# facebookresearch/VideoPose3D

Measured on NVIDIA H100. Metric: frames/sec (arc 3,3,3,3,3, T=243, N=1024), higher is better.
Workload: dtype fp16 (IEEE fp16 operands and activations, fp32 accumulate)

## Files before the change

videopose3d_b200/csrc/conv_gemm.cu:

```cuda
#include "conv_gemm.cuh"

#include <stdlib.h>
#include <string.h>

#include <type_traits>

#include "ptx.cuh"

namespace vp3d {

enum class Epi { kTrain, kGeneral, kLean };
enum class Fmt { kRuntime, kBf16, kF16, kI8 };
enum class Sched { kCooperative, kPingPong };
enum class U8Out { kNone, kBeside, kAlone };

struct InstKey {
  int block_n;
  Epi epi;
  Fmt fmt;
  Sched sched;
  bool res;
  bool out2;
  U8Out u8;
  constexpr bool operator==(const InstKey& o) const {
// ... 85 lines not shown
  const uint32_t q = quant_u8(v0, inv_s) | (quant_u8(v1, inv_s) << 8);
  asm volatile("st.shared.u16 [%0], %1;" ::"r"(addr), "h"((unsigned short)q) : "memory");
}

__device__ __forceinline__ void slab_reduce(float (&s)[8][2], float (&q)[8][2], float* s_pair,
                                            int lane, int wq, uint32_t bar_id) {
#pragma unroll
  for (int off = 4; off <= 16; off <<= 1) {
#pragma unroll
    for (int jj = 0; jj < 8; ++jj) {
#pragma unroll
      for (int e = 0; e < 2; ++e) {
        s[jj][e] += __shfl_xor_sync(0xffffffffu, s[jj][e], off);
        q[jj][e] += __shfl_xor_sync(0xffffffffu, q[jj][e], off);
      }
    }
  }
  if ((wq & 1) && lane < 4) {
#pragma unroll
    for (int jj = 0; jj < 8; ++jj) {
      *reinterpret_cast<float2*>(s_pair + 8 * jj + 2 * lane) = make_float2(s[jj][0], s[jj][1]);
      *reinterpret_cast<float2*>(s_pair + 64 + 8 * jj + 2 * lane) = make_float2(q[jj][0], q[jj][1]);
    }
  }
  named_bar_sync(bar_id, 64);
  if (!(wq & 1) && lane < 4) {
#pragma unroll
    for (int jj = 0; jj < 8; ++jj) {
      const float2 so = *reinterpret_cast<const float2*>(s_pair + 8 * jj + 2 * lane);
      const float2 qo = *reinterpret_cast<const float2*>(s_pair + 64 + 8 * jj + 2 * lane);
      s[jj][0] += so.x; s[jj][1] += so.y;
      q[jj][0] += qo.x; q[jj][1] += qo.y;
    }
  }
  named_bar_sync(bar_id, 64);
}

#ifdef VP3D_TIMELINE
__device__ __forceinline__ void tl_stamp(const ConvGemmArgs& p, int ev) {
  if (!p.timeline) return;
  int slot;
  if (blockIdx.x == 0) slot = 0;
  else if (blockIdx.x == gridDim.x - 1) slot = 1;
  else return;
  unsigned long long g;
  asm volatile("mov.u64 %0, %%globaltimer;" : "=l"(g));
  p.timeline[(slot * 32 + ev) * 2] = g;
  p.timeline[(slot * 32 + ev) * 2 + 1] = (unsigned long long)clock64();
}
#define TL(ev) tl_stamp(p, ev)
#else
#define TL(ev) ((void)0)
#endif

template <int BLOCK_N, Fmt FMT, int H, class Acc>
__device__ __forceinline__ void wgmma_kblock(Acc (&acc)[H][BLOCK_N / 2], const uint64_t (&da)[H],
                                             uint64_t db, bool first) {
#pragma unroll
  for (int h = 0; h < H; ++h) {
#pragma unroll
    for (int k = 0; k < 4; ++k) {
      const uint32_t accumulate = (first && k == 0) ? 0u : 1u;
      if constexpr (FMT == Fmt::kI8) {
        if constexpr (BLOCK_N == 128) wgmma_m64n128k32_u8s8(acc[h], da[h] + 2 * k, db + 2 * k, accumulate);
        else wgmma_m64n64k32_u8s8(acc[h], da[h] + 2 * k, db + 2 * k, accumulate);
      } else if constexpr (BLOCK_N == 128) {
        if constexpr (FMT == Fmt::kF16) wgmma_m64n128_f16(acc[h], da[h] + 2 * k, db + 2 * k, accumulate);
        else wgmma_m64n128_bf16(acc[h], da[h] + 2 * k, db + 2 * k, accumulate);
      } else {
        if constexpr (FMT == Fmt::kF16) wgmma_m64n64_f16(acc[h], da[h] + 2 * k, db + 2 * k, accumulate);
        else wgmma_m64n64_bf16(acc[h], da[h] + 2 * k, db + 2 * k, accumulate);
      }
    }
  }
}

template <class I, int H, class Issued>
__device__ __forceinline__ void mma_tile(typename I::Acc (&acc)[H][I::kBlockN / 2],
                                         const ConvGemmArgs& p, bool f16, uint32_t smem_a,
                                         uint32_t a_off, uint32_t smem_b, uint32_t full_bar,
                                         uint32_t empty_bar, uint32_t& stage_io, uint32_t& phase_io,
                                         int k_iters, int lane, bool tl_first, Issued issued) {
  uint32_t stage = stage_io, phase = phase_io;
  uint32_t prev_stage = 0;
  for (int it = 0; it < k_iters; ++it) {
    mbar_wait(full_bar + stage * 8, phase);
#ifdef VP3D_TIMELINE
    if (tl_first && it == 0) TL(4);
#endif
    const uint32_t a_st = smem_a + stage * I::kABytes + a_off;
    uint64_t da[H];
#pragma unroll
    for (int h = 0; h < H; ++h) da[h] = make_gmma_desc_sw128(a_st + h * 64 * 128, 16, 1024);
    const uint64_t db = make_gmma_desc_sw128(smem_b + stage * I::kBBytes, 16, 1024);
#pragma unroll
    for (int h = 0; h < H; ++h) wgmma_fence_operands(acc[h]);
    wgmma_fence();
    if constexpr (I::kFmt != Fmt::kRuntime) wgmma_kblock<I::kBlockN, I::kFmt>(acc, da, db, it == 0);
    else if (f16) wgmma_kblock<I::kBlockN, Fmt::kF16>(acc, da, db, it == 0);
    else wgmma_kblock<I::kBlockN, Fmt::kBf16>(acc, da, db, it == 0);
    wgmma_commit();
#pragma unroll
    for (int h = 0; h < H; ++h) wgmma_fence_operands(acc[h]);
    if (it > 0) {
      wgmma_wait<1>();
#pragma unroll
      for (int h = 0; h < H; ++h) wgmma_fence_operands(acc[h]);
      if (lane == 0) mbar_arrive(empty_bar + prev_stage * 8);
    }
    prev_stage = stage;
    if (++stage == I::kStages) { stage = 0; phase ^= 1; }
  }
  stage_io = stage; phase_io = phase;
  issued();
  wgmma_wait<0>();
#pragma unroll
  for (int h = 0; h < H; ++h) wgmma_fence_operands(acc[h]);
  if (k_iters > 0 && lane == 0) mbar_arrive(empty_bar + prev_stage * 8);
}

template <class I>
__global__ void __launch_bounds__(384, 1)
conv_gemm_kernel(const __grid_constant__ CUtensorMap tmap_a,
                 const __grid_constant__ CUtensorMap tmap_w,
                 const __grid_constant__ CUtensorMap tmap_out,
                 const __grid_constant__ CUtensorMap tmap_res,
                 const __grid_constant__ CUtensorMap tmap_z, const ConvGemmArgs p) {
  using Acc = typename I::Acc;
  constexpr int kBlocksPerTile = I::kBlockN / 64;
  constexpr int kFrag = I::kBlockN / 2;
  constexpr int kBK = I::kI8 ? kBlockK8 : kBlockK;

  extern __shared__ uint8_t smem_raw[];
  const uint32_t raw_addr = smem_u32(smem_raw);
  const uint32_t base = (raw_addr + 1023u) & ~1023u;
  uint8_t* smem = smem_raw + (base - raw_addr);

  const uint32_t smem_a = base;
  const uint32_t smem_b = base + I::kStages * I::kABytes;
  const uint32_t smem_store = base + I::kStages * I::kStageBytes;
  const uint32_t smem_res = smem_store + I::kStagingBytes;
  const uint32_t smem_u8 = smem_res + I::kResSlots * I::kTileBytes;
  const uint32_t bar_base = smem_u8 + I::kU8Bytes;
  const uint32_t full_bar = bar_base;
  const uint32_t empty_bar = bar_base + I::kStages * 8;
  const uint32_t rfull_bar = bar_base + 2 * I::kStages * 8;
  const uint32_t rempty_bar = rfull_bar + 32;
  const uint32_t dep_bar = rempty_bar + 32;
  const uint32_t affine_off = (dep_bar + 8 - base + 15u) & ~15u;
  float* s_affine = reinterpret_cast<float*>(smem + affine_off);
  float* s_pairs = reinterpret_cast<float*>(smem + affine_off + I::kAffineBytes);

  const int warp = threadIdx.x >> 5;
  const int lane = threadIdx.x & 31;
  if (threadIdx.x == 0) TL(0);

  const int m_tiles = p.dilated ? p.samples * p.tiles_per_sample : p.tiles_per_sample;
  const int total_tiles = m_tiles * p.n_tiles;
  const int k_iters = p.pairs * p.taps * p.kblocks_per_tap;
  const bool has_res = (p.flags & kEpiResidual) != 0;
  const bool bnb = I::kTrain && p.bnb != 0;
  const int aux_tiles = (has_res ? p.res_planes : 0) + (bnb ? 1 : 0);
  const int res_stages =
      (aux_tiles > 0 && I::kResSlots >= aux_tiles) ? I::kResSlots / aux_tiles : 1;

  if (warp == 0 && lane == 0) {
    tma_prefetch_desc(&tmap_a);
    tma_prefetch_desc(&tmap_w);
    tma_prefetch_desc(&tmap_out);
    if (I::kRes) tma_prefetch_desc(&tmap_res);
    if (I::kRes && bnb) tma_prefetch_desc(&tmap_z);
    if (I::kU8) tma_prefetch_desc(&tmap_z);
  }
  if (warp == 1 && lane == 0) {
    for (int s = 0; s < I::kStages; ++s) {
      mbar_init(full_bar + s * 8, 1);
      mbar_init(empty_bar + s * 8, I::kPP ? 4 : 8);
    }
    for (int s = 0; s < 4; ++s) {
      mbar_init(rfull_bar + s * 8, 1);
      mbar_init(rempty_bar + s * 8, I::kPP ? 1 : 256);
    }
    mbar_init(dep_bar, 1);
    fence_mbar_init();
  }
  __syncthreads();
  if (threadIdx.x == 0) TL(1);
  if (warp != 0) {
    griddep_wait();
    griddep_launch_dependents();
  }
  if (threadIdx.x == 32) {
    mbar_arrive(dep_bar);
    TL(2);
  }

  if (warp == 0) {
    if (lane == 0) {
      constexpr bool kEarlyW = !I::kTrain;
      if (!kEarlyW) mbar_wait(dep_bar, 0);
      const int n_pre = kEarlyW ? (k_iters < I::kStages ? k_iters : I::kStages) : 0;
      int mode = n_pre > 0 ? 0 : 2;
      if (kEarlyW && mode == 2) mbar_wait(dep_bar, 0);
      int w = blockIdx.x;
      if (w < total_tiles) {
        int n_blk, sample, row0;
        tile_coords(p, w, n_blk, sample, row0);
        uint32_t stage = 0, phase = 0;
        int it = 0, pair = 0, tap = 0, kb = 0;
        for (;;) {
          const int a_plane = (pair == 1) ? 1 : 0;
          const int w_plane = (pair == 2) ? 1 : 0;
          const uint32_t fb = full_bar + stage * 8;
          if (mode != 1) {
            mbar_wait(empty_bar + stage * 8, phase ^ 1);
            mbar_expect_tx(fb, I::kStageBytes);
            const int w_row = (w_plane * p.taps + tap) * p.n_pad + n_blk * I::kBlockN;
            tma_load_2d(&tmap_w, fb, smem_b + stage * I::kBBytes, kb * kBK, w_row);
          }
          if (mode != 0) {
            const int a_row = row0 + tap * p.tap_row_step;
            const int a_col = tap * p.tap_col_step + kb * kBK;
            tma_load_4d(&tmap_a, fb, smem_a + stage * I::kABytes, a_col, a_row, sample, a_plane);
#ifdef VP3D_TIMELINE
            if (w == (int)blockIdx.x && it == 0) TL(3);
#endif
          }
          if (++stage == I::kStages) { stage = 0; phase ^= 1; }
          ++it;
          if (++kb == p.kblocks_per_tap) {
            kb = 0;
            if (++tap == p.taps) { tap = 0; ++pair; }
          }
          if (mode == 0 && it == n_pre) {
            mbar_wait(dep_bar, 0);
            mode = 1;
            it = 0; pair = 0; tap = 0; kb = 0;
            stage = 0; phase = 0;
          } else if (mode == 1 && it == n_pre) {
            mode = 2;
          }
          if (it == k_iters) {
            w += gridDim.x;
            if (w >= total_tiles) break;
            tile_coords(p, w, n_blk, sample, row0);
            it = 0; pair = 0; tap = 0; kb = 0;
          }
        }
      }
    }
  } else if (warp == 1) {
    if (I::kPP && I::kRes && lane == 0) {
      uint32_t filled[2] = {0u, 0u};
      for (int j = 0, w = blockIdx.x; w < total_tiles; ++j, w += gridDim.x) {
        int n_blk, sample, row0;
        tile_coords(p, w, n_blk, sample, row0);
        const int g = j & 1;
        for (int sb = 0; sb < kBlocksPerTile; ++sb) {
          const uint32_t n = g ? filled[1] : filled[0];
          const uint32_t slot = 2u * g + (n & 1u);
          mbar_wait(rempty_bar + slot * 8, ((n >> 1) & 1u) ^ 1u);
          mbar_expect_tx(rfull_bar + slot * 8, I::kTileBytes);
          tma_load_4d(&tmap_res, rfull_bar + slot * 8, smem_res + slot * I::kTileBytes,
                      n_blk * I::kBlockN + sb * 64 + p.res_tma_col_off, row0 + p.res_tma_row_off,
                      sample, 0);
          if (g) ++filled[1];
          else ++filled[0];
        }
      }
    } else if (!I::kPP && I::kRes && lane == 0) {
      uint32_t rs = 0, rphase = 0;
      for (int w = blockIdx.x; w < total_tiles; w += gridDim.x) {
        int n_blk, sample, row0;
        tile_coords(p, w, n_blk, sample, row0);
        for (int sb = 0; sb < kBlocksPerTile; ++sb) {
          const int col = n_blk * I::kBlockN + sb * 64;
          const bool res_here = has_res && col >= p.res_col_begin && col < p.res_col_begin + p.res_cols;
          if (!res_here && !bnb) continue;
          const int n_res = res_here ? p.res_planes : 0;
          mbar_wait(rempty_bar + rs * 8, rphase ^ 1);
          mbar_expect_tx(rfull_bar + rs * 8, (n_res + (bnb ? 1 : 0)) * I::kTileBytes);
          const uint32_t slot0 = smem_res + rs * aux_tiles * I::kTileBytes;
          for (int pl = 0; pl < n_res; ++pl)
            tma_load_4d(&tmap_res, rfull_bar + rs * 8, slot0 + pl * I::kTileBytes,
                        col - p.res_col_begin + p.res_tma_col_off, row0 + p.res_tma_row_off, sample,
                        pl);
          if (bnb)
            tma_load_4d(&tmap_z, rfull_bar + rs * 8, slot0 + (aux_tiles - 1) * I::kTileBytes, col,
                        row0, sample, 0);
          if (++rs == (uint32_t)res_stages) { rs = 0; rphase ^= 1; }
        }
      }
    }
  } else if (I::kPP && warp >= 4) {
    const int wg = (warp - 4) >> 2;
    const int wq = warp & 3;
    const int tid = (int)threadIdx.x - 128 - 128 * wg;
    const int rl0 = 16 * wq + (lane >> 2);
    const int cq = 2 * (lane & 3);
    const uint32_t bar_wg = 2u + (uint32_t)wg;
    const uint32_t bar_mine = 8u + (uint32_t)wg, bar_other = 9u - (uint32_t)wg;
    const uint32_t staging = smem_store + wg * I::kTileBytes;
    uint32_t res_seen = 0;
    Acc acc[2][kFrag];
#pragma unroll
    for (int i = 0; i < kFrag; ++i) acc[0][i] = acc[1][i] = 0.0f;

    for (int j = wg, w = blockIdx.x + wg * gridDim.x; w < total_tiles; j += 2, w += 2 * gridDim.x) {
      int n_blk, sample, row0;
      tile_coords(p, w, n_blk, sample, row0);

      const uint32_t fill = (uint32_t)j * (uint32_t)k_iters;
      uint32_t stage = fill % I::kStages, phase = (fill / I::kStages) & 1u;
      if (j > 0) named_bar_sync(bar_mine, 256);
      mma_tile<I>(acc, p, I::kF16, smem_a, 0u, smem_b, full_bar, empty_bar, stage, phase, k_iters,
                  lane, warp == 4 && lane == 0 && w == (int)blockIdx.x, [&] {
                    if (w + (int)gridDim.x < total_tiles) named_bar_arrive(bar_other, 256);
                  });
#ifdef VP3D_TIMELINE
      if (warp == 4 && lane == 0) { if (w == (int)blockIdx.x) TL(7); TL(8); }
#endif

      const float* scale = p.scale + n_blk * I::kBlockN;
      const float* shift = p.shift + n_blk * I::kBlockN;
#pragma unroll
      for (int sb = 0; sb < kBlocksPerTile; ++sb) {
        const int cb = n_blk * I::kBlockN + sb * 64;
        uint32_t tile_smem;
        if constexpr (I::kRes) {
          const uint32_t slot = 2u * wg + (res_seen & 1u);
          mbar_wait(rfull_bar + slot * 8, (res_seen >> 1) & 1u);
          ++res_seen;
          tile_smem = smem_res + slot * I::kTileBytes;
          if constexpr (I::kU8) {
            if (tid == 0) tma_store_wait_read<0>();
            named_bar_sync(bar_wg, 128);
          }
        } else {
          if (tid == 0) tma_store_wait_read<0>();
          named_bar_sync(bar_wg, 128);
          tile_smem = staging;
        }
        const uint32_t u8_tile = I::kU8Alone ? staging : smem_u8 + (uint32_t)wg * (kBlockM * 64);
#pragma unroll
        for (int jj = 0; jj < 8; ++jj) {
          const int j4 = 4 * (sb * 8 + jj);
          const int cl = sb * 64 + jj * 8 + cq;
          const float2 sc = __ldg(reinterpret_cast<const float2*>(scale + cl));
          const float2 sh = __ldg(reinterpret_cast<const float2*>(shift + cl));
#pragma unroll
          for (int h2 = 0; h2 < 2; ++h2) {
#pragma unroll
            for (int h = 0; h < 2; ++h) {
              float v0 = fmaxf(fmaf(static_cast<float>(acc[h2][j4 + 2 * h]), sc.x, sh.x), 0.0f);
              float v1 = fmaxf(fmaf(static_cast<float>(acc[h2][j4 + 2 * h + 1]), sc.y, sh.y), 0.0f);
              const uint32_t off = sw128_off(64 * h2 + rl0 + 8 * h, jj * 8 + cq);
              if (I::kRes) add_pair(v0, v1, ld_shared_u32(tile_smem + off), I::kF16);
              if constexpr (I::kStore16)
                st_shared_u32(tile_smem + off, I::kF16 ? pack_f16x2(v0, v1) : pack_bf16x2(v0, v1));
              if constexpr (I::kU8)
                st_u8_pair(u8_tile + (uint32_t)(64 * h2 + rl0 + 8 * h) * 64u + jj * 8 + cq, v0, v1,
                           p.u8_inv_s);
            }
          }
        }
        fence_proxy_async_smem();
        named_bar_sync(bar_wg, 128);
        if (tid == 0) {
#pragma unroll
          for (int hb = 0; hb < 4; ++hb) {
            if constexpr (I::kStore16)
              tma_store_4d(&tmap_out, tile_smem + hb * 4096u, cb, row0 + 32 * hb, sample, 0);
            if constexpr (I::kU8)
              tma_store_4d(&tmap_z, u8_tile + hb * 2048u, cb, row0 + 32 * hb, sample, 0);
          }
          tma_store_commit();
        }
      }
      if (I::kRes && tid == 0) {
        tma_store_wait_read<0>();
#pragma unroll
        for (int sb = 0; sb < kBlocksPerTile; ++sb)
          mbar_arrive(rempty_bar + (2u * wg + ((res_seen - kBlocksPerTile + sb) & 1u)) * 8);
      }
#ifdef VP3D_TIMELINE
      if (warp == 4 && lane == 0) { if (w == (int)blockIdx.x) TL(9); TL(10); }
#endif
    }
    if (tid == 0) tma_store_wait_all<0>();
#ifdef VP3D_TIMELINE
    if (warp == 4 && lane == 0) TL(11);
#endif
  } else if (!I::kPP && warp >= 4) {
    const int wg = (warp - 4) >> 2;
    const int wq = warp & 3;
    const int tid = (int)threadIdx.x - 128 - 128 * wg;
    const int rl0 = 16 * wq + (lane >> 2);
    const int cq = 2 * (lane & 3);
    const uint32_t bar_wg = 2u + (uint32_t)wg;
    const uint32_t bar_slab = 4u + (uint32_t)(wg * 2 + (wq >> 1));
    float* s_pair = s_pairs + (wg * 2 + (wq >> 1)) * 128;
    const bool f16 = I::kLean ? I::kF16 : p.f16 != 0;
    const bool do_relu = I::kLean || (p.flags & kEpiRelu);
    const bool do_res = I::kLean ? I::kRes : (p.flags & kEpiResidual) != 0;
    const bool do_stats = I::kTrain && (p.flags & kEpiStats);
    const bool do_f32 = !I::kLean && (p.flags & kEpiOutF32);
    const bool do_affine = I::kLean || (p.flags & kEpiAffine);
    const bool two_planes = I::kOut2 && p.out_planes == 2;
    uint32_t stage = 0, phase = 0;
    uint32_t ablock = 0;
    uint32_t sbuf = 0;
    int aff_n_blk = -1;
    Acc acc[1][kFrag];
#pragma unroll
    for (int i = 0; i < kFrag; ++i) acc[0][i] = 0.0f;

    for (int w = blockIdx.x; w < total_tiles; w += gridDim.x) {
      int n_blk, sample, row0;
      tile_coords(p, w, n_blk, sample, row0);
      const int m_blk = w / p.n_tiles;

      mma_tile<I>(acc, p, f16, smem_a, wg * 64 * 128, smem_b, full_bar, empty_bar, stage, phase,
                  k_iters, lane, warp == 4 && lane == 0 && w == (int)blockIdx.x, [] {});
#ifdef VP3D_TIMELINE
      if (warp == 4 && lane == 0) { if (w == (int)blockIdx.x) TL(7); TL(8); }
#endif

      if (do_affine && n_blk != aff_n_blk) {
        named_bar_sync(1, 256);
        const int e = (int)threadIdx.x - 128;
        if (e < I::kBlockN) {
          s_affine[e] = __ldg(p.scale + n_blk * I::kBlockN + e);
          s_affine[I::kBlockN + e] = __ldg(p.shift + n_blk * I::kBlockN + e);
        }
        named_bar_sync(1, 256);
        aff_n_blk = n_blk;
      }

      int t_in[2];
      bool valid[2];
      long long out_row[2], res_row[2];
      bool res_ok[2];
#pragma unroll
      for (int h = 0; h < 2; ++h) {
        const int rt = 64 * wg + rl0 + 8 * h;
        t_in[h] = row0 + rt;
        valid[h] = t_in[h] < p.out_rows;
        out_row[h] = (long long)sample * p.out_rows + t_in[h];
        res_row[h] = 0;
        res_ok[h] = valid[h];
        if (!I::kRes) {
          int rsmp = sample, rtt = t_in[h];
          if (!p.dilated && p.res_sample_div > 0) {
            rsmp = t_in[h] / p.res_sample_div;
            rtt = t_in[h] - rsmp * p.res_sample_div;
          }
          const long long in_sample = (long long)rtt * p.res_row_step + p.res_row_off;
          if (p.res_check_rows && (in_sample < 0 || in_sample >= p.res_rows_per_sample)) res_ok[h] = false;
          res_row[h] = (long long)rsmp * p.res_rows_per_sample + in_sample;
        }
      }
      const bool two_planes_t =
          two_planes && (p.dilated || (row0 < p.lo_row_end && row0 + kBlockM > p.lo_row_begin));

#pragma unroll
      for (int sb = 0; sb < kBlocksPerTile; ++sb) {
        const int cb = n_blk * I::kBlockN + sb * 64;
        const bool res_here = do_res && cb >= p.res_col_begin && cb < p.res_col_begin + p.res_cols;
        const bool aux_here = I::kRes && (res_here || bnb);
        const uint32_t rs = aux_here ? ablock % (uint32_t)res_stages : 0u;
        const uint32_t rphase = aux_here ? (ablock / (uint32_t)res_stages) & 1u : 0u;
        if (aux_here) {
          ++ablock;
          mbar_wait(rfull_bar + rs * 8, rphase);
        }
        const uint32_t aux0 = smem_res + (rs * aux_tiles) * I::kTileBytes;
        const uint32_t my_store = smem_store + (wg * 2 + sbuf) * (I::kOut2 ? 2 : 1) * I::kHalfBytes;
        const uint32_t my_u8 = I::kU8Alone ? my_store : smem_u8 + (uint32_t)(wg * 2 + sbuf) * (64 * 64);
        if (!do_f32) {
          if (tid == 0) tma_store_wait_read<1>();
          named_bar_sync(bar_wg, 128);
        }
        float ss[8][2], sq[8][2];
#pragma unroll
        for (int jj = 0; jj < 8; ++jj) {
          const int j = sb * 8 + jj;
          const int cl = sb * 64 + jj * 8 + cq;
          const int c = cb + jj * 8 + cq;
          float v[2][2] = {{static_cast<float>(acc[0][4 * j]), static_cast<float>(acc[0][4 * j + 1])},
                           {static_cast<float>(acc[0][4 * j + 2]), static_cast<float>(acc[0][4 * j + 3])}};
          if (do_affine) {
            const float2 sc = *reinterpret_cast<const float2*>(s_affine + cl);
            const float2 sh = *reinterpret_cast<const float2*>(s_affine + I::kBlockN + cl);
#pragma unroll
            for (int h = 0; h < 2; ++h) {
              v[h][0] = fmaf(v[h][0], sc.x, sh.x);
              v[h][1] = fmaf(v[h][1], sc.y, sh.y);
            }
          }
          if (do_relu) {
#pragma unroll
            for (int h = 0; h < 2; ++h) { v[h][0] = fmaxf(v[h][0], 0.0f); v[h][1] = fmaxf(v[h][1], 0.0f); }
          }
          if (I::kRes) {
            if (res_here) {
#pragma unroll
              for (int h = 0; h < 2; ++h) {
                const uint32_t off = sw128_off(64 * wg + rl0 + 8 * h, jj * 8 + cq);
                add_pair(v[h][0], v[h][1], ld_shared_u32(aux0 + off), f16);
                for (int pl = 1; pl < p.res_planes; ++pl)
                  add_pair(v[h][0], v[h][1], ld_shared_u32(aux0 + pl * I::kTileBytes + off), false);
              }
            }
          } else if (res_here) {
#pragma unroll
            for (int h = 0; h < 2; ++h) {
              if (!res_ok[h]) continue;
              const __nv_bfloat16* rp = p.res + res_row[h] * p.res_ld + (c - p.res_col_begin);
#pragma unroll
              for (int pl = 0; pl < 2; ++pl) {
                if (pl < p.res_planes) {
                  const uint32_t u = __ldg(reinterpret_cast<const unsigned int*>(rp + pl * p.res_plane_stride));
                  add_pair(v[h][0], v[h][1], u, f16 && pl == 0);
                }
              }
            }
          }
          if (do_f32) {
#pragma unroll
            for (int h = 0; h < 2; ++h) {
              if (!valid[h]) continue;
              float* op = p.out_f32 + out_row[h] * p.out_f32_ld + c;
              if (c < p.n_valid) op[0] = v[h][0];
              if (c + 1 < p.n_valid) op[1] = v[h][1];
            }
          } else {
            if constexpr (I::kU8) {
#pragma unroll
              for (int h = 0; h < 2; ++h)
                st_u8_pair(my_u8 + (uint32_t)(rl0 + 8 * h) * 64u + jj * 8 + cq, v[h][0], v[h][1],
                           p.u8_inv_s);
            }
#pragma unroll
            for (int h = 0; h < 2 && I::kStore16; ++h) {
              const uint32_t hi = f16 ? pack_f16x2(v[h][0], v[h][1]) : pack_bf16x2(v[h][0], v[h][1]);
              const uint32_t off = sw128_off(rl0 + 8 * h, jj * 8 + cq);
              st_shared_u32(my_store + off, hi);
              if (two_planes_t) {
                const uint32_t lo = pack_bf16x2(v[h][0] - bf16_lo_to_f(hi), v[h][1] - bf16_hi_to_f(hi));
                st_shared_u32(my_store + I::kHalfBytes + off, lo);
              }
            }
          }
          if (I::kRes && bnb) {
            const int ch = c % p.bnb_c;
            const bool drop = p.bnb_p > 0.0f;
            const uint32_t thresh = (uint32_t)(p.bnb_p * 65536.0f);
            const float inv_keep = drop ? 1.0f / (1.0f - p.bnb_p) : 1.0f;
            ss[jj][0] = ss[jj][1] = sq[jj][0] = sq[jj][1] = 0.0f;
#pragma unroll
            for (int h = 0; h < 2; ++h) {
              const uint32_t zu =
                  ld_shared_u32(aux0 + (aux_tiles - 1) * I::kTileBytes + sw128_off(64 * wg + rl0 + 8 * h, jj * 8 + cq));
              const float z2[2] = {bf16_lo_to_f(zu), bf16_hi_to_f(zu)};
              const int c0 = c & ~31;
              const unsigned long long elem0 = (unsigned long long)out_row[h] * p.out_ld + c0;
              const uint32_t key = p.bnb_seed_lo ^ (p.bnb_seed_hi * 0x7F4A7C15u) ^
                                   (p.bnb_layer * 0x632BE5ABu) ^
                                   ((uint32_t)((elem0 >> 1) >> 32) * 0x85EBCA77u);
              float m[2] = {1.0f, 1.0f};
              if (drop) {
                uint32_t hh = ((uint32_t)(elem0 >> 1) + (uint32_t)((c - c0) >> 1)) * 0x9E3779B1u + key;
                hh ^= hh >> 16; hh *= 0x85EBCA6Bu; hh ^= hh >> 13; hh *= 0xC2B2AE35u; hh ^= hh >> 16;
                m[0] = ((hh & 0xFFFFu) >= thresh) ? inv_keep : 0.0f;
                m[1] = ((hh >> 16) >= thresh) ? inv_keep : 0.0f;
              }
#pragma unroll
              for (int e = 0; e < 2; ++e) {
                const float g = __bfloat162float(__float2bfloat16_rn(v[h][e]));
                const float y = fmaf(z2[e], __ldg(p.bnb_scale + ch + e), __ldg(p.bnb_shift + ch + e));
                float dy = (valid[h] && y > 0.0f) ? g : 0.0f;
                dy *= m[e];
                ss[jj][e] += dy;
                sq[jj][e] += dy * (z2[e] - __ldg(p.bnb_mean + ch + e));
              }
            }
          } else if (do_stats) {
#pragma unroll
            for (int e = 0; e < 2; ++e) {
              const float x0 = valid[0] ? v[0][e] : 0.0f;
              const float x1 = valid[1] ? v[1][e] : 0.0f;
              ss[jj][e] = x0 + x1;
              sq[jj][e] = x0 * x0 + x1 * x1;
            }
          }
        }
        if (I::kRes && aux_here) mbar_arrive(rempty_bar + rs * 8);
        if (I::kTrain && ((I::kRes && bnb) || do_stats)) {
          slab_reduce(ss, sq, s_pair, lane, wq, bar_slab);
          if (!(wq & 1) && lane < 4) {
            float* sp = ((I::kRes && bnb) ? p.bnb_sums : p.stats) +
                        ((size_t)(m_blk * 4 + 2 * wg + (wq >> 1)) * 2) * p.n_pad + cb + 2 * lane;
#pragma unroll
            for (int jj = 0; jj < 8; ++jj) {
              sp[8 * jj] = ss[jj][0];
              sp[8 * jj + 1] = ss[jj][1];
              sp[p.n_pad + 8 * jj] = sq[jj][0];
              sp[p.n_pad + 8 * jj + 1] = sq[jj][1];
            }
          }
        }
        if (!do_f32) {
          fence_proxy_async_smem();
          named_bar_sync(bar_wg, 128);
          if (tid == 0) {
#pragma unroll
            for (int hb = 0; hb < 2; ++hb) {
              const int r = row0 + 64 * wg + 32 * hb;
              if constexpr (I::kStore16) tma_store_4d(&tmap_out, my_store + hb * 4096u, cb, r, sample, 0);
              if constexpr (I::kU8) tma_store_4d(&tmap_z, my_u8 + hb * 2048u, cb, r, sample, 0);
              if (two_planes_t) tma_store_4d(&tmap_out, my_store + I::kHalfBytes + hb * 4096u, cb, r, sample, 1);
            }
            tma_store_commit();
          }
          sbuf ^= 1u;
        }
      }
#ifdef VP3D_TIMELINE
      if (warp == 4 && lane == 0) { if (w == (int)blockIdx.x) TL(9); TL(10); }
#endif
    }
    if (tid == 0) tma_store_wait_all<0>();
#ifdef VP3D_TIMELINE
    if (warp == 4 && lane == 0) TL(11);
#endif
  }
}

static int g_pdl = -1;
static bool pdl_enabled() {
  if (g_pdl < 0) {
    const char* e = getenv("VP3D_PDL");
    g_pdl = (e && e[0] == '0') ? 0 : 1;
  }
  return g_pdl != 0;
}
void conv_gemm_set_pdl(int on) { g_pdl = on ? 1 : 0; }
bool conv_gemm_pdl_enabled() { return pdl_enabled(); }

static int conv_tiles(const ConvGemmArgs& a) {
  const int m_tiles = a.dilated ? a.samples * a.tiles_per_sample : a.tiles_per_sample;
  return m_tiles * a.n_tiles;
}

template <class I>
static cudaError_t launch_impl(const CUtensorMap& tmap_a, const CUtensorMap& tmap_w,
                               const CUtensorMap& tmap_out, const CUtensorMap& tmap_res,
                               const CUtensorMap& tmap_z, const ConvGemmArgs& args, int num_sms,
                               cudaStream_t stream) {
  auto kernel = conv_gemm_kernel<I>;
  static bool attr_set[kMaxDevices] = {};
  int dev = 0;
  cudaError_t e = cudaGetDevice(&dev);
  if (e != cudaSuccess) return e;
  if (dev < 0 || dev >= kMaxDevices) return cudaErrorInvalidDevice;
  if (!attr_set[dev]) {
    e = cudaFuncSetAttribute(kernel, cudaFuncAttributeMaxDynamicSharedMemorySize, I::kSmemBytes);
    if (e != cudaSuccess) return e;
    attr_set[dev] = true;
  }
  const int total = conv_tiles(args);
  if (total <= 0) return cudaSuccess;
  const int workers = total < num_sms ? total : num_sms;
  cudaLaunchConfig_t cfg;
  memset(&cfg, 0, sizeof(cfg));
  cfg.gridDim = dim3(workers, 1, 1);
  cfg.blockDim = dim3(384, 1, 1);
  cfg.dynamicSmemBytes = I::kSmemBytes;
  cfg.stream = stream;
  cudaLaunchAttribute attr[1];
  int n_attr = 0;
  if (pdl_enabled()) {
    attr[n_attr].id = cudaLaunchAttributeProgrammaticStreamSerialization;
    attr[n_attr].val.programmaticStreamSerializationAllowed = 1;
    ++n_attr;
  }
// ... 106 lines not shown
```

videopose3d_b200/csrc/ptx.cuh:

```cuda
#pragma once
#include <cuda.h>
#include <cuda_bf16.h>
#include <cuda_fp16.h>
#include <cuda_runtime.h>
#include <stdint.h>

namespace vp3d {

#ifndef VP3D_SPIN_LIMIT
#define VP3D_SPIN_LIMIT (1u << 27)
#endif

__device__ __forceinline__ uint32_t smem_u32(const void* p) {
  return static_cast<uint32_t>(__cvta_generic_to_shared(p));
}

__device__ __forceinline__ void griddep_wait() {
  asm volatile("griddepcontrol.wait;" ::: "memory");
}
__device__ __forceinline__ void griddep_launch_dependents() {
  asm volatile("griddepcontrol.launch_dependents;" ::: "memory");
}

__device__ __forceinline__ void mbar_init(uint32_t bar, uint32_t count) {
  asm volatile("mbarrier.init.shared::cta.b64 [%0], %1;" ::"r"(bar), "r"(count) : "memory");
}
__device__ __forceinline__ void fence_mbar_init() {
  asm volatile("fence.mbarrier_init.release.cluster;" ::: "memory");
}
__device__ __forceinline__ void mbar_expect_tx(uint32_t bar, uint32_t bytes) {
  asm volatile("mbarrier.arrive.expect_tx.shared::cta.b64 _, [%0], %1;" ::"r"(bar), "r"(bytes)
               : "memory");
}
__device__ __forceinline__ void mbar_arrive(uint32_t bar) {
  asm volatile("mbarrier.arrive.shared::cta.b64 _, [%0];" ::"r"(bar) : "memory");
}
__device__ __forceinline__ bool mbar_try_wait(uint32_t bar, uint32_t parity) {
  uint32_t ok;
  asm volatile(
      "{\n\t.reg .pred P;\n\t"
      "mbarrier.try_wait.parity.shared::cta.b64 P, [%1], %2;\n\t"
      "selp.u32 %0, 1, 0, P;\n\t}"
      : "=r"(ok)
      : "r"(bar), "r"(parity)
      : "memory");
  return ok != 0;
}
__device__ __forceinline__ void mbar_wait(uint32_t bar, uint32_t parity) {
  uint32_t spins = 0;
  while (!mbar_try_wait(bar, parity)) {
    if (++spins > VP3D_SPIN_LIMIT) __trap();
  }
}

__device__ __forceinline__ void tma_prefetch_desc(const CUtensorMap* m) {
  asm volatile("prefetch.tensormap [%0];" ::"l"(reinterpret_cast<uint64_t>(m)) : "memory");
}
__device__ __forceinline__ void tma_load_2d(const CUtensorMap* m, uint32_t bar, uint32_t dst,
                                            int c0, int c1) {
  asm volatile(
      "cp.async.bulk.tensor.2d.shared::cluster.global.mbarrier::complete_tx::bytes"
      " [%0], [%1, {%3, %4}], [%2];"
      ::"r"(dst), "l"(reinterpret_cast<uint64_t>(m)), "r"(bar), "r"(c0), "r"(c1)
      : "memory");
}
__device__ __forceinline__ void tma_load_4d(const CUtensorMap* m, uint32_t bar, uint32_t dst,
                                            int c0, int c1, int c2, int c3) {
  asm volatile(
      "cp.async.bulk.tensor.4d.shared::cluster.global.mbarrier::complete_tx::bytes"
      " [%0], [%1, {%3, %4, %5, %6}], [%2];"
      ::"r"(dst), "l"(reinterpret_cast<uint64_t>(m)), "r"(bar), "r"(c0), "r"(c1), "r"(c2), "r"(c3)
      : "memory");
}
__device__ __forceinline__ void tma_store_4d(const CUtensorMap* m, uint32_t src, int c0, int c1,
                                             int c2, int c3) {
  asm volatile(
      "cp.async.bulk.tensor.4d.global.shared::cta.bulk_group [%0, {%2, %3, %4, %5}], [%1];"
      ::"l"(reinterpret_cast<uint64_t>(m)), "r"(src), "r"(c0), "r"(c1), "r"(c2), "r"(c3)
      : "memory");
}
__device__ __forceinline__ void tma_store_commit() {
  asm volatile("cp.async.bulk.commit_group;" ::: "memory");
}
template <int N>
__device__ __forceinline__ void tma_store_wait_read() {
  asm volatile("cp.async.bulk.wait_group.read %0;" ::"n"(N) : "memory");
}
template <int N>
__device__ __forceinline__ void tma_store_wait_all() {
  asm volatile("cp.async.bulk.wait_group %0;" ::"n"(N) : "memory");
}
__device__ __forceinline__ void fence_proxy_async_smem() {
  asm volatile("fence.proxy.async.shared::cta;" ::: "memory");
}
__device__ __forceinline__ void named_bar_sync(uint32_t id, uint32_t count) {
  asm volatile("bar.sync %0, %1;" ::"r"(id), "r"(count) : "memory");
}
__device__ __forceinline__ void named_bar_arrive(uint32_t id, uint32_t count) {
  asm volatile("bar.arrive %0, %1;" ::"r"(id), "r"(count) : "memory");
}

__device__ __forceinline__ uint64_t make_gmma_desc_sw128(uint32_t smem_addr, uint32_t lbo_bytes,
                                                         uint32_t sbo_bytes) {
  uint64_t d = 0;
  d |= static_cast<uint64_t>((smem_addr & 0x3FFFFu) >> 4);
  d |= static_cast<uint64_t>((lbo_bytes >> 4) & 0x3FFFu) << 16;
  d |= static_cast<uint64_t>((sbo_bytes >> 4) & 0x3FFFu) << 32;
  d |= static_cast<uint64_t>(1) << 62;
  return d;
}
__device__ __forceinline__ void wgmma_fence() {
  asm volatile("wgmma.fence.sync.aligned;" ::: "memory");
}
__device__ __forceinline__ void wgmma_commit() {
  asm volatile("wgmma.commit_group.sync.aligned;" ::: "memory");
}
template <int N>
__device__ __forceinline__ void wgmma_wait() {
  asm volatile("wgmma.wait_group.sync.aligned %0;" ::"n"(N) : "memory");
}
template <int R>
__device__ __forceinline__ void wgmma_fence_operands(float (&d)[R]) {
#pragma unroll
  for (int i = 0; i < R; ++i) asm volatile("" : "+f"(d[i])::"memory");
}

__device__ __forceinline__ void wgmma_m64n64_bf16(float (&d)[32], uint64_t da, uint64_t db,
                                                  uint32_t accumulate) {
  asm volatile(
      "{\n\t.reg .pred p;\n\tsetp.ne.b32 p, %34, 0;\n\t"
      "wgmma.mma_async.sync.aligned.m64n64k16.f32.bf16.bf16 {%0, %1, %2, %3, %4, %5, %6, %7, %8, %9, %10, %11, %12, %13, %14, %15, %16, %17, %18, %19, %20, %21, %22, %23, %24, %25, %26, %27, %28, %29, %30, %31}, %32, %33, p, 1, 1, 0, 0;\n\t}"
      : "+f"(d[0]), "+f"(d[1]), "+f"(d[2]), "+f"(d[3]), "+f"(d[4]), "+f"(d[5]), "+f"(d[6]), "+f"(d[7]), "+f"(d[8]), "+f"(d[9]), "+f"(d[10]), "+f"(d[11]), "+f"(d[12]), "+f"(d[13]), "+f"(d[14]), "+f"(d[15]), "+f"(d[16]), "+f"(d[17]), "+f"(d[18]), "+f"(d[19]), "+f"(d[20]), "+f"(d[21]), "+f"(d[22]), "+f"(d[23]), "+f"(d[24]), "+f"(d[25]), "+f"(d[26]), "+f"(d[27]), "+f"(d[28]), "+f"(d[29]), "+f"(d[30]), "+f"(d[31])
      : "l"(da), "l"(db), "r"(accumulate));
}

__device__ __forceinline__ void wgmma_m64n64_f16(float (&d)[32], uint64_t da, uint64_t db,
                                                  uint32_t accumulate) {
  asm volatile(
      "{\n\t.reg .pred p;\n\tsetp.ne.b32 p, %34, 0;\n\t"
      "wgmma.mma_async.sync.aligned.m64n64k16.f32.f16.f16 {%0, %1, %2, %3, %4, %5, %6, %7, %8, %9, %10, %11, %12, %13, %14, %15, %16, %17, %18, %19, %20, %21, %22, %23, %24, %25, %26, %27, %28, %29, %30, %31}, %32, %33, p, 1, 1, 0, 0;\n\t}"
      : "+f"(d[0]), "+f"(d[1]), "+f"(d[2]), "+f"(d[3]), "+f"(d[4]), "+f"(d[5]), "+f"(d[6]), "+f"(d[7]), "+f"(d[8]), "+f"(d[9]), "+f"(d[10]), "+f"(d[11]), "+f"(d[12]), "+f"(d[13]), "+f"(d[14]), "+f"(d[15]), "+f"(d[16]), "+f"(d[17]), "+f"(d[18]), "+f"(d[19]), "+f"(d[20]), "+f"(d[21]), "+f"(d[22]), "+f"(d[23]), "+f"(d[24]), "+f"(d[25]), "+f"(d[26]), "+f"(d[27]), "+f"(d[28]), "+f"(d[29]), "+f"(d[30]), "+f"(d[31])
      : "l"(da), "l"(db), "r"(accumulate));
}

__device__ __forceinline__ void wgmma_m64n64_bf16_mn(float (&d)[32], uint64_t da, uint64_t db,
                                                  uint32_t accumulate) {
  asm volatile(
      "{\n\t.reg .pred p;\n\tsetp.ne.b32 p, %34, 0;\n\t"
      "wgmma.mma_async.sync.aligned.m64n64k16.f32.bf16.bf16 {%0, %1, %2, %3, %4, %5, %6, %7, %8, %9, %10, %11, %12, %13, %14, %15, %16, %17, %18, %19, %20, %21, %22, %23, %24, %25, %26, %27, %28, %29, %30, %31}, %32, %33, p, 1, 1, 1, 1;\n\t}"
      : "+f"(d[0]), "+f"(d[1]), "+f"(d[2]), "+f"(d[3]), "+f"(d[4]), "+f"(d[5]), "+f"(d[6]), "+f"(d[7]), "+f"(d[8]), "+f"(d[9]), "+f"(d[10]), "+f"(d[11]), "+f"(d[12]), "+f"(d[13]), "+f"(d[14]), "+f"(d[15]), "+f"(d[16]), "+f"(d[17]), "+f"(d[18]), "+f"(d[19]), "+f"(d[20]), "+f"(d[21]), "+f"(d[22]), "+f"(d[23]), "+f"(d[24]), "+f"(d[25]), "+f"(d[26]), "+f"(d[27]), "+f"(d[28]), "+f"(d[29]), "+f"(d[30]), "+f"(d[31])
      : "l"(da), "l"(db), "r"(accumulate));
}

__device__ __forceinline__ void wgmma_m64n128_bf16(float (&d)[64], uint64_t da, uint64_t db,
                                                  uint32_t accumulate) {
  asm volatile(
      "{\n\t.reg .pred p;\n\tsetp.ne.b32 p, %66, 0;\n\t"
      "wgmma.mma_async.sync.aligned.m64n128k16.f32.bf16.bf16 {%0, %1, %2, %3, %4, %5, %6, %7, %8, %9, %10, %11, %12, %13, %14, %15, %16, %17, %18, %19, %20, %21, %22, %23, %24, %25, %26, %27, %28, %29, %30, %31, %32, %33, %34, %35, %36, %37, %38, %39, %40, %41, %42, %43, %44, %45, %46, %47, %48, %49, %50, %51, %52, %53, %54, %55, %56, %57, %58, %59, %60, %61, %62, %63}, %64, %65, p, 1, 1, 0, 0;\n\t}"
      : "+f"(d[0]), "+f"(d[1]), "+f"(d[2]), "+f"(d[3]), "+f"(d[4]), "+f"(d[5]), "+f"(d[6]), "+f"(d[7]), "+f"(d[8]), "+f"(d[9]), "+f"(d[10]), "+f"(d[11]), "+f"(d[12]), "+f"(d[13]), "+f"(d[14]), "+f"(d[15]), "+f"(d[16]), "+f"(d[17]), "+f"(d[18]), "+f"(d[19]), "+f"(d[20]), "+f"(d[21]), "+f"(d[22]), "+f"(d[23]), "+f"(d[24]), "+f"(d[25]), "+f"(d[26]), "+f"(d[27]), "+f"(d[28]), "+f"(d[29]), "+f"(d[30]), "+f"(d[31]), "+f"(d[32]), "+f"(d[33]), "+f"(d[34]), "+f"(d[35]), "+f"(d[36]), "+f"(d[37]), "+f"(d[38]), "+f"(d[39]), "+f"(d[40]), "+f"(d[41]), "+f"(d[42]), "+f"(d[43]), "+f"(d[44]), "+f"(d[45]), "+f"(d[46]), "+f"(d[47]), "+f"(d[48]), "+f"(d[49]), "+f"(d[50]), "+f"(d[51]), "+f"(d[52]), "+f"(d[53]), "+f"(d[54]), "+f"(d[55]), "+f"(d[56]), "+f"(d[57]), "+f"(d[58]), "+f"(d[59]), "+f"(d[60]), "+f"(d[61]), "+f"(d[62]), "+f"(d[63])
      : "l"(da), "l"(db), "r"(accumulate));
}

__device__ __forceinline__ void wgmma_m64n128_f16(float (&d)[64], uint64_t da, uint64_t db,
                                                  uint32_t accumulate) {
  asm volatile(
      "{\n\t.reg .pred p;\n\tsetp.ne.b32 p, %66, 0;\n\t"
      "wgmma.mma_async.sync.aligned.m64n128k16.f32.f16.f16 {%0, %1, %2, %3, %4, %5, %6, %7, %8, %9, %10, %11, %12, %13, %14, %15, %16, %17, %18, %19, %20, %21, %22, %23, %24, %25, %26, %27, %28, %29, %30, %31, %32, %33, %34, %35, %36, %37, %38, %39, %40, %41, %42, %43, %44, %45, %46, %47, %48, %49, %50, %51, %52, %53, %54, %55, %56, %57, %58, %59, %60, %61, %62, %63}, %64, %65, p, 1, 1, 0, 0;\n\t}"
      : "+f"(d[0]), "+f"(d[1]), "+f"(d[2]), "+f"(d[3]), "+f"(d[4]), "+f"(d[5]), "+f"(d[6]), "+f"(d[7]), "+f"(d[8]), "+f"(d[9]), "+f"(d[10]), "+f"(d[11]), "+f"(d[12]), "+f"(d[13]), "+f"(d[14]), "+f"(d[15]), "+f"(d[16]), "+f"(d[17]), "+f"(d[18]), "+f"(d[19]), "+f"(d[20]), "+f"(d[21]), "+f"(d[22]), "+f"(d[23]), "+f"(d[24]), "+f"(d[25]), "+f"(d[26]), "+f"(d[27]), "+f"(d[28]), "+f"(d[29]), "+f"(d[30]), "+f"(d[31]), "+f"(d[32]), "+f"(d[33]), "+f"(d[34]), "+f"(d[35]), "+f"(d[36]), "+f"(d[37]), "+f"(d[38]), "+f"(d[39]), "+f"(d[40]), "+f"(d[41]), "+f"(d[42]), "+f"(d[43]), "+f"(d[44]), "+f"(d[45]), "+f"(d[46]), "+f"(d[47]), "+f"(d[48]), "+f"(d[49]), "+f"(d[50]), "+f"(d[51]), "+f"(d[52]), "+f"(d[53]), "+f"(d[54]), "+f"(d[55]), "+f"(d[56]), "+f"(d[57]), "+f"(d[58]), "+f"(d[59]), "+f"(d[60]), "+f"(d[61]), "+f"(d[62]), "+f"(d[63])
      : "l"(da), "l"(db), "r"(accumulate));
}

template <int R>
__device__ __forceinline__ void wgmma_fence_operands(int (&d)[R]) {
#pragma unroll
  for (int i = 0; i < R; ++i) asm volatile("" : "+r"(d[i])::"memory");
}

__device__ __forceinline__ void wgmma_m64n64k32_u8s8(int (&d)[32], uint64_t da, uint64_t db,
                                                      uint32_t accumulate) {
  asm volatile(
      "{\n\t.reg .pred p;\n\tsetp.ne.b32 p, %34, 0;\n\t"
      "wgmma.mma_async.sync.aligned.m64n64k32.s32.u8.s8 {%0, %1, %2, %3, %4, %5, %6, %7, %8, %9, %10, %11, %12, %13, %14, %15, %16, %17, %18, %19, %20, %21, %22, %23, %24, %25, %26, %27, %28, %29, %30, %31}, %32, %33, p;\n\t}"
      : "+r"(d[0]), "+r"(d[1]), "+r"(d[2]), "+r"(d[3]), "+r"(d[4]), "+r"(d[5]), "+r"(d[6]), "+r"(d[7]), "+r"(d[8]), "+r"(d[9]), "+r"(d[10]), "+r"(d[11]), "+r"(d[12]), "+r"(d[13]), "+r"(d[14]), "+r"(d[15]), "+r"(d[16]), "+r"(d[17]), "+r"(d[18]), "+r"(d[19]), "+r"(d[20]), "+r"(d[21]), "+r"(d[22]), "+r"(d[23]), "+r"(d[24]), "+r"(d[25]), "+r"(d[26]), "+r"(d[27]), "+r"(d[28]), "+r"(d[29]), "+r"(d[30]), "+r"(d[31])
      : "l"(da), "l"(db), "r"(accumulate));
}

__device__ __forceinline__ void wgmma_m64n128k32_u8s8(int (&d)[64], uint64_t da, uint64_t db,
                                                       uint32_t accumulate) {
  asm volatile(
      "{\n\t.reg .pred p;\n\tsetp.ne.b32 p, %66, 0;\n\t"
      "wgmma.mma_async.sync.aligned.m64n128k32.s32.u8.s8 {%0, %1, %2, %3, %4, %5, %6, %7, %8, %9, %10, %11, %12, %13, %14, %15, %16, %17, %18, %19, %20, %21, %22, %23, %24, %25, %26, %27, %28, %29, %30, %31, %32, %33, %34, %35, %36, %37, %38, %39, %40, %41, %42, %43, %44, %45, %46, %47, %48, %49, %50, %51, %52, %53, %54, %55, %56, %57, %58, %59, %60, %61, %62, %63}, %64, %65, p;\n\t}"
      : "+r"(d[0]), "+r"(d[1]), "+r"(d[2]), "+r"(d[3]), "+r"(d[4]), "+r"(d[5]), "+r"(d[6]), "+r"(d[7]), "+r"(d[8]), "+r"(d[9]), "+r"(d[10]), "+r"(d[11]), "+r"(d[12]), "+r"(d[13]), "+r"(d[14]), "+r"(d[15]), "+r"(d[16]), "+r"(d[17]), "+r"(d[18]), "+r"(d[19]), "+r"(d[20]), "+r"(d[21]), "+r"(d[22]), "+r"(d[23]), "+r"(d[24]), "+r"(d[25]), "+r"(d[26]), "+r"(d[27]), "+r"(d[28]), "+r"(d[29]), "+r"(d[30]), "+r"(d[31]), "+r"(d[32]), "+r"(d[33]), "+r"(d[34]), "+r"(d[35]), "+r"(d[36]), "+r"(d[37]), "+r"(d[38]), "+r"(d[39]), "+r"(d[40]), "+r"(d[41]), "+r"(d[42]), "+r"(d[43]), "+r"(d[44]), "+r"(d[45]), "+r"(d[46]), "+r"(d[47]), "+r"(d[48]), "+r"(d[49]), "+r"(d[50]), "+r"(d[51]), "+r"(d[52]), "+r"(d[53]), "+r"(d[54]), "+r"(d[55]), "+r"(d[56]), "+r"(d[57]), "+r"(d[58]), "+r"(d[59]), "+r"(d[60]), "+r"(d[61]), "+r"(d[62]), "+r"(d[63])
      : "l"(da), "l"(db), "r"(accumulate));
}

__device__ __forceinline__ uint32_t quant_u8(float v, float inv_s) {
  uint32_t q;
  asm("cvt.rni.sat.u8.f32 %0, %1;" : "=r"(q) : "f"(v * inv_s));
  return q;
}

__device__ __forceinline__ void wgmma_m64n128_bf16_mn(float (&d)[64], uint64_t da, uint64_t db,
                                                  uint32_t accumulate) {
  asm volatile(
      "{\n\t.reg .pred p;\n\tsetp.ne.b32 p, %66, 0;\n\t"
      "wgmma.mma_async.sync.aligned.m64n128k16.f32.bf16.bf16 {%0, %1, %2, %3, %4, %5, %6, %7, %8, %9, %10, %11, %12, %13, %14, %15, %16, %17, %18, %19, %20, %21, %22, %23, %24, %25, %26, %27, %28, %29, %30, %31, %32, %33, %34, %35, %36, %37, %38, %39, %40, %41, %42, %43, %44, %45, %46, %47, %48, %49, %50, %51, %52, %53, %54, %55, %56, %57, %58, %59, %60, %61, %62, %63}, %64, %65, p, 1, 1, 1, 1;\n\t}"
      : "+f"(d[0]), "+f"(d[1]), "+f"(d[2]), "+f"(d[3]), "+f"(d[4]), "+f"(d[5]), "+f"(d[6]), "+f"(d[7]), "+f"(d[8]), "+f"(d[9]), "+f"(d[10]), "+f"(d[11]), "+f"(d[12]), "+f"(d[13]), "+f"(d[14]), "+f"(d[15]), "+f"(d[16]), "+f"(d[17]), "+f"(d[18]), "+f"(d[19]), "+f"(d[20]), "+f"(d[21]), "+f"(d[22]), "+f"(d[23]), "+f"(d[24]), "+f"(d[25]), "+f"(d[26]), "+f"(d[27]), "+f"(d[28]), "+f"(d[29]), "+f"(d[30]), "+f"(d[31]), "+f"(d[32]), "+f"(d[33]), "+f"(d[34]), "+f"(d[35]), "+f"(d[36]), "+f"(d[37]), "+f"(d[38]), "+f"(d[39]), "+f"(d[40]), "+f"(d[41]), "+f"(d[42]), "+f"(d[43]), "+f"(d[44]), "+f"(d[45]), "+f"(d[46]), "+f"(d[47]), "+f"(d[48]), "+f"(d[49]), "+f"(d[50]), "+f"(d[51]), "+f"(d[52]), "+f"(d[53]), "+f"(d[54]), "+f"(d[55]), "+f"(d[56]), "+f"(d[57]), "+f"(d[58]), "+f"(d[59]), "+f"(d[60]), "+f"(d[61]), "+f"(d[62]), "+f"(d[63])
      : "l"(da), "l"(db), "r"(accumulate));
}


__device__ __forceinline__ uint32_t pack_bf16x2(float lo, float hi) {
  __nv_bfloat162 v = __floats2bfloat162_rn(lo, hi);
  return *reinterpret_cast<uint32_t*>(&v);
}
__device__ __forceinline__ uint32_t pack_f16x2(float lo, float hi) {
  uint32_t r;
  asm("cvt.rn.satfinite.f16x2.f32 %0, %1, %2;" : "=r"(r) : "f"(hi), "f"(lo));
  return r;
}
__device__ __forceinline__ float f16_lo_to_f(uint32_t v) {
  return __half2float(__ushort_as_half(static_cast<unsigned short>(v & 0xFFFFu)));
}
__device__ __forceinline__ float f16_hi_to_f(uint32_t v) {
  return __half2float(__ushort_as_half(static_cast<unsigned short>(v >> 16)));
}
__device__ __forceinline__ float bf16_lo_to_f(uint32_t v) { return __uint_as_float(v << 16); }
__device__ __forceinline__ float bf16_hi_to_f(uint32_t v) { return __uint_as_float(v & 0xFFFF0000u); }

}
```

Baseline: 1.408 million.

## Use ldmatrix/stmatrix for residual epilogue and defer residual slot release

In the ping-pong epilogue's residual path, the per-element 32-bit shared loads and stores of the swizzled residual tile are replaced with ldmatrix.x4/stmatrix.x4, cutting shared-memory instruction count. Releasing the residual buffer slots (waiting on TMA store reads and arriving on rempty barriers) moves from the end of each tile to just before the next tile's MMA. This keeps the store-read wait off the epilogue's critical path. The risk is that slots are released later, which can delay the residual prefetch producer, and that the hand-computed ldmatrix address and swizzle mapping must match the existing layout exactly.

After: 1.413 million (median of 6 runs). No clear change (+0.4%).

```diff
diff --git a/videopose3d_b200/csrc/conv_gemm.cu b/videopose3d_b200/csrc/conv_gemm.cu
--- a/videopose3d_b200/csrc/conv_gemm.cu
+++ b/videopose3d_b200/csrc/conv_gemm.cu
@@ -411,6 +411,8 @@
     const uint32_t bar_mine = 8u + (uint32_t)wg, bar_other = 9u - (uint32_t)wg;
     const uint32_t staging = smem_store + wg * I::kTileBytes;
     uint32_t res_seen = 0;
+    const uint32_t mrow = 16u * wq + 8u * ((lane >> 3) & 1) + (lane & 7);
+    const uint32_t mchunk = (uint32_t)(lane >> 4) ^ (uint32_t)(lane & 7);
     Acc acc[2][kFrag];
 #pragma unroll
     for (int i = 0; i < kFrag; ++i) acc[0][i] = acc[1][i] = 0.0f;
@@ -421,7 +423,15 @@
 
       const uint32_t fill = (uint32_t)j * (uint32_t)k_iters;
       uint32_t stage = fill % I::kStages, phase = (fill / I::kStages) & 1u;
-      if (j > 0) named_bar_sync(bar_mine, 256);
+      if (j > 0) {
+        if (I::kRes && j >= 2 && tid == 0) {
+          tma_store_wait_read<0>();
+#pragma unroll
+          for (int sb = 0; sb < kBlocksPerTile; ++sb)
+            mbar_arrive(rempty_bar + (2u * wg + ((res_seen - kBlocksPerTile + sb) & 1u)) * 8);
+        }
+        named_bar_sync(bar_mine, 256);
+      }
       mma_tile<I>(acc, p, I::kF16, smem_a, 0u, smem_b, full_bar, empty_bar, stage, phase, k_iters,
                   lane, warp == 4 && lane == 0 && w == (int)blockIdx.x, [&] {
                     if (w + (int)gridDim.x < total_tiles) named_bar_arrive(bar_other, 256);
@@ -432,65 +442,93 @@
 
       const float* scale = p.scale + n_blk * I::kBlockN;
       const float* shift = p.shift + n_blk * I::kBlockN;
+      auto epi_rows = [&](int sb, uint32_t tile_smem, uint32_t u8_pair) {
+#pragma unroll
+        for (int q = 0; q < 4; ++q) {
+          float2 sc[2], sh[2];
+#pragma unroll
+          for (int e = 0; e < 2; ++e) {
+            const int cl = sb * 64 + (2 * q + e) * 8 + cq;
+            sc[e] = *reinterpret_cast<const float2*>(scale + cl);
+            sh[e] = *reinterpret_cast<const float2*>(shift + cl);
+          }
+#pragma unroll
+          for (int h2 = 0; h2 < 2; ++h2) {
+            const uint32_t addr = tile_smem + (64u * h2 + mrow) * 128u + ((mchunk ^ (2u * q)) << 4);
+            uint32_t r[4];
+            if constexpr (I::kRes) ldmatrix_x4(addr, r);
+#pragma unroll
+            for (int i = 0; i < 4; ++i) {
+              const int h = i & 1, e = i >> 1;
+              const int j4 = 4 * (sb * 8 + 2 * q + e) + 2 * h;
+              float v0 = fmaxf(fmaf(static_cast<float>(acc[h2][j4]), sc[e].x, sh[e].x), 0.0f);
+              float v1 = fmaxf(fmaf(static_cast<float>(acc[h2][j4 + 1]), sc[e].y, sh[e].y), 0.0f);
+              if constexpr (I::kRes) add_pair(v0, v1, r[i], I::kF16);
+              r[i] = I::kF16 ? pack_f16x2(v0, v1) : pack_bf16x2(v0, v1);
+              if constexpr (I::kU8)
+                st_u8_pair(u8_pair + (uint32_t)(64 * h2 + 8 * h) * 64u + (2 * q + e) * 8, v0, v1,
+                           p.u8_inv_s);
+            }
+            if constexpr (I::kStore16) stmatrix_x4(addr, r);
+          }
+        }
+      };
+      const uint32_t u8_tile = I::kU8Alone ? staging : smem_u8 + (uint32_t)wg * (kBlockM * 64);
+      const uint32_t u8_mine = u8_tile + (uint32_t)rl0 * 64u + cq;
+      auto store_tile = [&](int sb, uint32_t tile_smem) {
+        const int cb = n_blk * I::kBlockN + sb * 64;
+#pragma unroll
+        for (int hb = 0; hb < 4; ++hb) {
+          if constexpr (I::kStore16)
+            tma_store_4d(&tmap_out, tile_smem + hb * 4096u, cb, row0 + 32 * hb, sample, 0);
+          if constexpr (I::kU8)
+            tma_store_4d(&tmap_z, u8_tile + hb * 2048u, cb, row0 + 32 * hb, sample, 0);
+        }
+        tma_store_commit();
+      };
 #pragma unroll
       for (int sb = 0; sb < kBlocksPerTile; ++sb) {
-        const int cb = n_blk * I::kBlockN + sb * 64;
-        uint32_t tile_smem;
         if constexpr (I::kRes) {
           const uint32_t slot = 2u * wg + (res_seen & 1u);
           mbar_wait(rfull_bar + slot * 8, (res_seen >> 1) & 1u);
           ++res_seen;
-          tile_smem = smem_res + slot * I::kTileBytes;
+          const uint32_t tile_smem = smem_res + slot * I::kTileBytes;
           if constexpr (I::kU8) {
             if (tid == 0) tma_store_wait_read<0>();
             named_bar_sync(bar_wg, 128);
           }
+          epi_rows(sb, tile_smem, u8_mine);
+          fence_proxy_async_smem();
+          named_bar_sync(bar_wg, 128);
+          if (tid == 0) store_tile(sb, tile_smem);
         } else {
           if (tid == 0) tma_store_wait_read<0>();
           named_bar_sync(bar_wg, 128);
-          tile_smem = staging;
-        }
-        const uint32_t u8_tile = I::kU8Alone ? staging : smem_u8 + (uint32_t)wg * (kBlockM * 64);
-#pragma unroll
-        for (int jj = 0; jj < 8; ++jj) {
-          const int j4 = 4 * (sb * 8 + jj);
-          const int cl = sb * 64 + jj * 8 + cq;
-          const float2 sc = __ldg(reinterpret_cast<const float2*>(scale + cl));
-          const float2 sh = __ldg(reinterpret_cast<const float2*>(shift + cl));
-#pragma unroll
-          for (int h2 = 0; h2 < 2; ++h2) {
-#pragma unroll
-            for (int h = 0; h < 2; ++h) {
-              float v0 = fmaxf(fmaf(static_cast<float>(acc[h2][j4 + 2 * h]), sc.x, sh.x), 0.0f);
-              float v1 = fmaxf(fmaf(static_cast<float>(acc[h2][j4 + 2 * h + 1]), sc.y, sh.y), 0.0f);
-              const uint32_t off = sw128_off(64 * h2 + rl0 + 8 * h, jj * 8 + cq);
-              if (I::kRes) add_pair(v0, v1, ld_shared_u32(tile_smem + off), I::kF16);
-              if constexpr (I::kStore16)
-                st_shared_u32(tile_smem + off, I::kF16 ? pack_f16x2(v0, v1) : pack_bf16x2(v0, v1));
-              if constexpr (I::kU8)
-                st_u8_pair(u8_tile + (uint32_t)(64 * h2 + rl0 + 8 * h) * 64u + jj * 8 + cq, v0, v1,
-                           p.u8_inv_s);
-            }
-          }
-        }
-        fence_proxy_async_smem();
-        named_bar_sync(bar_wg, 128);
-        if (tid == 0) {
-#pragma unroll
-          for (int hb = 0; hb < 4; ++hb) {
-            if constexpr (I::kStore16)
-              tma_store_4d(&tmap_out, tile_smem + hb * 4096u, cb, row0 + 32 * hb, sample, 0);
-            if constexpr (I::kU8)
-              tma_store_4d(&tmap_z, u8_tile + hb * 2048u, cb, row0 + 32 * hb, sample, 0);
-          }
-          tma_store_commit();
-        }
-      }
-      if (I::kRes && tid == 0) {
-        tma_store_wait_read<0>();
-#pragma unroll
-        for (int sb = 0; sb < kBlocksPerTile; ++sb)
-          mbar_arrive(rempty_bar + (2u * wg + ((res_seen - kBlocksPerTile + sb) & 1u)) * 8);
+#pragma unroll
+          for (int jj = 0; jj < 8; ++jj) {
+            const int j4 = 4 * (sb * 8 + jj);
+            const int cl = sb * 64 + jj * 8 + cq;
+            const float2 sc = __ldg(reinterpret_cast<const float2*>(scale + cl));
+            const float2 sh = __ldg(reinterpret_cast<const float2*>(shift + cl));
+#pragma unroll
+            for (int h2 = 0; h2 < 2; ++h2) {
+#pragma unroll
+              for (int h = 0; h < 2; ++h) {
+                float v0 = fmaxf(fmaf(static_cast<float>(acc[h2][j4 + 2 * h]), sc.x, sh.x), 0.0f);
+                float v1 = fmaxf(fmaf(static_cast<float>(acc[h2][j4 + 2 * h + 1]), sc.y, sh.y), 0.0f);
+                const uint32_t off = sw128_off(64 * h2 + rl0 + 8 * h, jj * 8 + cq);
+                if constexpr (I::kStore16)
+                  st_shared_u32(staging + off, I::kF16 ? pack_f16x2(v0, v1) : pack_bf16x2(v0, v1));
+                if constexpr (I::kU8)
+                  st_u8_pair(u8_tile + (uint32_t)(64 * h2 + rl0 + 8 * h) * 64u + jj * 8 + cq, v0, v1,
+                             p.u8_inv_s);
+              }
+            }
+          }
+          fence_proxy_async_smem();
+          named_bar_sync(bar_wg, 128);
+          if (tid == 0) store_tile(sb, staging);
+        }
       }
 #ifdef VP3D_TIMELINE
       if (warp == 4 && lane == 0) { if (w == (int)blockIdx.x) TL(9); TL(10); }
diff --git a/videopose3d_b200/csrc/ptx.cuh b/videopose3d_b200/csrc/ptx.cuh
--- a/videopose3d_b200/csrc/ptx.cuh
+++ b/videopose3d_b200/csrc/ptx.cuh
@@ -92,6 +92,14 @@
 }
 __device__ __forceinline__ void fence_proxy_async_smem() {
   asm volatile("fence.proxy.async.shared::cta;" ::: "memory");
+}
+__device__ __forceinline__ void stmatrix_x4(uint32_t addr, const uint32_t (&r)[4]) {
+  asm volatile("stmatrix.sync.aligned.m8n8.x4.shared.b16 [%0], {%1, %2, %3, %4};"
+               ::"r"(addr), "r"(r[0]), "r"(r[1]), "r"(r[2]), "r"(r[3]) : "memory");
+}
+__device__ __forceinline__ void ldmatrix_x4(uint32_t addr, uint32_t (&r)[4]) {
+  asm volatile("ldmatrix.sync.aligned.m8n8.x4.shared.b16 {%0, %1, %2, %3}, [%4];"
+               : "=r"(r[0]), "=r"(r[1]), "=r"(r[2]), "=r"(r[3]) : "r"(addr) : "memory");
 }
 __device__ __forceinline__ void named_bar_sync(uint32_t id, uint32_t count) {
   asm volatile("bar.sync %0, %1;" ::"r"(id), "r"(count) : "memory");
```
